# AiRyunn/BoT

Hardware: AMD Instinct MI355X
Metric: edges/sec full-batch GAT fwd+bwd on ogbn-arxiv; achieved HBM GB/s vs peak (higher is better)
Workload: dtype f32

## Files before the change

bot_amd/_C.py:

```python
from __future__ import annotations

import ctypes
import os
from ctypes import c_char_p, c_double, c_float, c_int32, c_int64, c_uint64, c_void_p

import torch

_HERE = os.path.dirname(os.path.abspath(__file__))
LIB_PATH = os.environ.get("BOT_AMD_LIB") or os.path.join(_HERE, "lib", "libbot_gnn.so")
ABI_VERSION = 19

if not os.path.exists(LIB_PATH):
    raise ImportError(
        f"{LIB_PATH} is missing: build the gfx950 kernels first "
        "(`make -C bot_amd/csrc` or `python -c 'import __graft_entry__ as g; g.build()'`). "
        "bot_amd has no CPU / PyTorch fallback."
    )
_lib = ctypes.CDLL(LIB_PATH)

_P = c_void_p
_SIGS = {
    "bot_abi_version": (ctypes.c_int, []),
    "bot_last_error": (c_char_p, []),
    "bot_last_kernel": (c_char_p, []),
# ... 88 lines not shown
                                                c_uint64, _P, _P, _P, c_double, _P, c_int64, _P, _P]),
    "bot_halves_tn_combine_f32": (ctypes.c_int, [_P, _P, c_int32, c_int32, c_int32, c_int32, _P, _P, _P, c_int64, _P]),
    "bot_halves_scale_from_slots2_f32": (ctypes.c_int, [_P, c_float, _P, c_float, _P, _P]),
    "bot_halves_tail_f16": (ctypes.c_int, [c_int64, c_int32, _P, _P, _P, _P, _P, c_int64, c_int32, _P]),
    "bot_spmm_dot_halves_fits": (ctypes.c_int, [_P, c_int64, c_int64, _P, c_int64, c_int64, c_int32, c_int32, _P, c_int64, c_int64, c_int32]),
    "bot_spmm_dot_halves_f16": (ctypes.c_int, [_P, _P, c_int64, c_int64, _P, c_int64, _P, _P, c_int64, _P, c_int64, c_int64, _P, _P, _P, c_int64, c_int64,
                                               c_int32, c_int32, _P, _P, c_int64, c_int64, c_int32, _P, _P, _P]),
    "bot_gemm_halves3_nt_bn_rows": (c_int32, [c_int64]),
    "bot_gemm_halves3_nt3_f32": (ctypes.c_int, [c_int64, c_int64, c_int64, _P, _P, c_int64, _P, _P, c_int64, c_int64, _P, c_int64, c_int64, c_int32, _P, c_int64,
                                                _P, c_int32, _P]),
    "bot_gemm_halves3_nt_bn_deferred_max_k": (c_int32, []),
    "bot_gemm_halves3_nt_bn_reduce_f32": (ctypes.c_int, [c_int64, c_int64, c_int64, _P, _P, c_int64, _P, _P, c_int64, c_int64, _P, c_int64, c_int64, c_int32, _P, c_int64,
                                                         _P, _P]),
    "bot_gemm_halves3_nt_bn_apply_f32": (ctypes.c_int, [c_int64, c_int64, c_int64, _P, _P, c_int64, _P, _P, c_int64, c_int64, _P, c_int64, c_int64, c_int32, _P,
                                                        _P, _P, c_double, _P, c_int64, _P, _P, c_int64, c_int32, c_int32, c_int32, _P, _P]),
    "bot_bn_act_bwd_reduce_partials_f32": (ctypes.c_int, [_P, c_int32, c_int32, _P, _P, _P]),
    "bot_bn_bwd_bound_partials_f32": (ctypes.c_int, [c_int32, _P, c_int32, _P, _P, c_double, _P, _P, _P, _P]),
    "bot_bn_bwd_partials_finish_f32": (ctypes.c_int, [_P, _P, c_int32, c_int32, _P, _P, c_int32, c_double, _P, _P, _P, _P]),
    "bot_gemm_halves3_nt2_f32": (ctypes.c_int, [c_int64, c_int64, c_int64, _P, _P, c_int64, _P, _P, c_int64, c_int64, _P, c_int64, c_int64, c_int32, _P, c_int64,
                                                c_int32, _P]),
    "bot_halves_split_frag_f16": (ctypes.c_int, [_P, c_int64, c_int64, c_int32, _P, _P, c_int32, _P]),
    "bot_gemm_halves3_tn2_f32": (ctypes.c_int, [c_int64, c_int64, c_int64, c_int64, c_int64, _P, _P, _P, c_int64, _P, c_int64, c_int64, _P, c_int64, c_int64, _P,
                                                c_int64, _P, c_int32, _P]),
    "bot_stream_create": (ctypes.c_int, [c_int32, _P]),
    "bot_gemm_halves3_nt_grouped2_f32": (ctypes.c_int, [c_int64, c_int64, _P, _P, _P, c_int64, c_int64, _P, c_int64, c_int64, _P, c_int64, c_int32, _P,
                                                        c_int32, _P, _P, c_int32, _P, _P, _P, _P, c_int32, c_int32, _P]),
    "bot_bn_stats_halves_partials_f32": (ctypes.c_int, [_P, _P, c_int32, _P, c_int64, c_int32, c_float, c_float, _P, _P, _P, _P, _P, _P, _P, c_float, _P, _P, _P]),
    "bot_absmax_slots": (c_int32, []),
    "bot_absmax_slots_f32": (ctypes.c_int, [_P, c_int64, c_int64, c_int32, _P, _P]),
    "bot_halves_scale_from_slots_f32": (ctypes.c_int, [_P, _P, _P]),
# ... 841 lines not shown
        n = b.shape[0]
    if out is None:
        out = torch.empty((m, n), dtype=torch.float32, device=a.device)
    st = None
    if bn is not None:
        if not bn.fits(m, n, k):
            raise BotKernelError("gemm_halves3_nt: this product cannot carry the BatchNorm-backward by-product (BnBwdStats.fits)")
        st = bn.struct()
    _check(_timed("gemm_halves", (m, n, 3 * k, 1), lambda: _lib.bot_gemm_halves3_nt3_f32(
        m, n, k, scale_a.data_ptr(), _ptr(scale_a2), int(k_split), scale_b.data_ptr(), a.data_ptr(), _ld(a), 2 * piece_a if a2_off is None else a2_off,
        b.data_ptr(), _ld(b), piece_b, int(bool(b_frag)), out.data_ptr(), _ld(out), ctypes.addressof(st) if st is not None else None, int(mode), _stream())),
        "gemm_halves3_nt")
    return out


def dh_deferred_max_k() -> int:
    return int(_lib.bot_gemm_halves3_nt_bn_deferred_max_k())


def gemm_halves3_nt_bn_reduce(a, b, scale_a, scale_b, piece_b, k, bn, a2_off, scale_a2=None, k_split=0, b_frag=False, n=None, out=None):
    _dev(a, b, scale_a, scale_b, scale_a2, out)
    m = a.shape[0]
    n = b.shape[0] if n is None else n
    st = bn.struct()
    _check(_timed("gemm_halves", (m, n, 3 * k, 1), lambda: _lib.bot_gemm_halves3_nt_bn_reduce_f32(
        m, n, k, scale_a.data_ptr(), _ptr(scale_a2), int(k_split), scale_b.data_ptr(), a.data_ptr(), _ld(a), a2_off, b.data_ptr(), _ld(b), piece_b,
        int(bool(b_frag)), _ptr(out), _ld(out) if out is not None else 0, ctypes.addressof(st), _stream())), "gemm_halves3_nt_bn_reduce")


def gemm_halves3_nt_bn_apply(a, b, scale_a, scale_b, piece_b, k, bn, a2_off, sum_g, sum_gx, total_count, scale_a2=None, k_split=0, b_frag=False, n=None,
# ... 813 lines not shown
```

bot_amd/csrc/dense.hip:

```cpp
#include <hip/hip_fp16.h>

#include "common.h"

#include <stdlib.h>

namespace bot {

constexpr int kTX = 64;
constexpr int kTY = 4;
constexpr int kRowBlocks = 256;

template <int VEC>
__device__ __forceinline__ void drop_factors(uint64_t seed, int64_t r, int c, int64_t nquad, float p, float scale, float (&f)[VEC]) {
    uint32_t w[4];
    Philox::gen(seed, (uint64_t)(r * nquad + (c >> 2)), w);
#pragma unroll
    for (int t = 0; t < VEC; ++t) f[t] = ((w[(c & 3) + t] >> 8) * (1.0f / 16777216.0f)) >= p ? scale : 0.f;
}

template <int VEC>
__device__ __forceinline__ void load_cols(float (&v)[VEC], const float* p, bool wide, int nv) {
    if constexpr (VEC == 4) {
        if (wide && nv == 4) {
            vload<4>(v, p);
        } else {
            const float2 a = *reinterpret_cast<const float2*>(p);
            v[0] = a.x, v[1] = a.y, v[2] = 0.f, v[3] = 0.f;
            if (nv == 4) {
                const float2 b = *reinterpret_cast<const float2*>(p + 2);
                v[2] = b.x, v[3] = b.y;
            }
        }
    } else {
        vload<VEC>(v, p);
    }
}
template <int VEC>
__device__ __forceinline__ void store_cols(float* p, const float (&v)[VEC], bool wide, int nv) {
    if constexpr (VEC == 4) {
        if (wide && nv == 4) {
            vstore<4>(p, v);
        } else {
            *reinterpret_cast<float2*>(p) = make_float2(v[0], v[1]);
            if (nv == 4) *reinterpret_cast<float2*>(p + 2) = make_float2(v[2], v[3]);
        }
    } else {
        vstore<VEC>(p, v);
    }
}
template <int VEC>
__device__ __forceinline__ void load_param(float (&v)[VEC], const float* a, int c, int F, float dflt) {
#pragma unroll
    for (int t = 0; t < VEC; ++t) v[t] = (a && c + t < F) ? a[c + t] : dflt;
}

__device__ __forceinline__ uint64_t eff_seed(uint64_t seed, const uint64_t* off) {
    return off ? seed + off[0] * 0x9E3779B97F4A7C15ull : seed;
}

struct BnArgs {
    const float* x;
    int64_t ldx;
    int64_t n;
    int32_t F;
    const float* mean;
    const float* invstd;
    const float* w;
    const float* b;
    int32_t relu;
    float p;
    uint64_t seed;
    const uint64_t* seed_offset;
    __half* hout;
    int32_t hpieces;
// ... 267 lines not shown
    const int64_t step = (int64_t)gridDim.y * kTY;
    for (int64_t r0 = (int64_t)blockIdx.y * kTY + ty; r0 < a.n; r0 += step * UR) {
        float v[UR][VEC];
#pragma unroll
        for (int u = 0; u < UR; ++u) {
            const int64_t r = r0 + u * step;
            if (r < a.n) load_cols<VEC>(v[u], a.x + r * a.ldx + c, a.wx, nv);
        }
#pragma unroll
        for (int u = 0; u < UR; ++u) {
            const int64_t r = r0 + u * step;
            if (r >= a.n) break;
            float f[VEC];
            if (a.p > 0.f) drop_factors<VEC>(seed, r, c, nquad, a.p, scale, f);
#pragma unroll
            for (int t = 0; t < VEC; ++t) {
                float o = fmaf(v[u][t] - mu[t], sc[t], sh[t]);
                if (a.relu) o = fmaxf(o, 0.f);
                if (a.p > 0.f) o *= f[t];
                v[u][t] = o;
            }
            if (a.y) store_cols<VEC>(a.y + r * a.ldy + c, v[u], a.wy, nv);
            if constexpr (VEC == 4) {
                if (a.hout) {
                    __half h1[4], h2[4];
#pragma unroll
                    for (int t = 0; t < 4; ++t) {
                        const float z = t < nv ? v[u][t] * hs : 0.f;
                        h1[t] = __float2half_rn(z);
                        h2[t] = __float2half_rn((z - __half2float(h1[t])) * kHalvesShift);
                    }
                    __half* o = a.hout + r * a.ldh + c;
                    const uint2 hi = *reinterpret_cast<const uint2*>(h1), lo = *reinterpret_cast<const uint2*>(h2);
                    *reinterpret_cast<uint2*>(o) = hi;
                    if (a.hpieces == 3) *reinterpret_cast<uint2*>(o + a.piece) = hi, *reinterpret_cast<uint2*>(o + 2 * (int64_t)a.piece) = lo;
                    else *reinterpret_cast<uint2*>(o + a.piece) = lo;
                }
            }
        }
    }
}

constexpr int kRowSeg = 8;
__global__ __launch_bounds__(256) void bn_act_fwd_rowseg_kernel(BnArgs a) {
    const int c = threadIdx.x * 4;
    if (c >= a.piece) return;
// ... 12 lines not shown
    const uint64_t seed = eff_seed(a.seed, a.seed_offset);
    const int64_t r0 = (int64_t)blockIdx.x * kRowSeg;
    float v[kRowSeg][4];
#pragma unroll
    for (int u = 0; u < kRowSeg; ++u)
        if (live && r0 + u < a.n) load_cols<4>(v[u], a.x + (r0 + u) * a.ldx + c, a.wx, nv);
#pragma unroll
    for (int u = 0; u < kRowSeg; ++u) {
        const int64_t r = r0 + u;
        if (r >= a.n) break;
        __half h1[4], h2[4];
        float f[4];
        if (live && a.p > 0.f) drop_factors<4>(seed, r, c, nquad, a.p, scale, f);
#pragma unroll
        for (int t = 0; t < 4; ++t) {
            float o = 0.f;
            if (t < nv) {
                o = fmaf(v[u][t] - mu[t], sc[t], sh[t]);
                if (a.relu) o = fmaxf(o, 0.f);
                if (a.p > 0.f) o *= f[t];
            }
            const float z = o * hs;
            h1[t] = __float2half_rn(z);
            h2[t] = __float2half_rn((z - __half2float(h1[t])) * kHalvesShift);
            v[u][t] = o;
        }
        if (a.y && live) store_cols<4>(a.y + r * a.ldy + c, v[u], a.wy, nv);
        __half* o = a.hout + r * a.ldh + c;
        const uint2 hi = *reinterpret_cast<const uint2*>(h1), lo = *reinterpret_cast<const uint2*>(h2);
        *reinterpret_cast<uint2*>(o) = hi;
        if (a.hpieces == 3) *reinterpret_cast<uint2*>(o + a.piece) = hi, *reinterpret_cast<uint2*>(o + 2 * (int64_t)a.piece) = lo;
        else *reinterpret_cast<uint2*>(o + a.piece) = lo;
    }
}

template <int VEC>
__global__ __launch_bounds__(kTX* kTY) void bn_act_bwd_reduce_kernel(BnArgs a) {
    __shared__ float lds[2][kTY][kTX * VEC];
    const int tx = threadIdx.x % kTX, ty = threadIdx.x / kTX;
// ... 605 lines not shown
```

bot_amd/csrc/halves3.hip:

```cpp
#include <hip/hip_fp16.h>

#include <stdlib.h>
#include <string.h>

#include <algorithm>
#include <type_traits>
#include <utility>

#include "common.h"

namespace bot {
namespace {

constexpr int BK = 32;

typedef _Float16 half8 __attribute__((ext_vector_type(8)));
typedef float f32x4 __attribute__((ext_vector_type(4)));

struct H3Args {
    const _Float16* A;
    const _Float16* B;
    const float* scale_a;
    const float* scale_b;
    float* C;
// ... 749 lines not shown
                    if (e < b_nv) pm[e] = b_gm[e], pm[F + e] = b_xm[e];
            }
        }
    }
}

__global__ __launch_bounds__(512) void gemm_halves3_nt64_kernel(H3Args p) { gemm_halves3_nt64_body<false, false>(p, nullptr); }
__global__ __launch_bounds__(512) void gemm_halves3_nt64_frag_kernel(H3Args p) { gemm_halves3_nt64_body<false, true>(p, nullptr); }
__global__ __launch_bounds__(512) void gemm_halves3_nt64_grouped_kernel(H3Args p, H3Groups groups) { gemm_halves3_nt64_body<true, false>(p, &groups); }
__global__ __launch_bounds__(512) void gemm_halves3_nt64_bnb_kernel(H3Args p) { gemm_halves3_nt64_body<false, false, kBnbStore>(p, nullptr); }
__global__ __launch_bounds__(512) void gemm_halves3_nt64_frag_bnb_kernel(H3Args p) { gemm_halves3_nt64_body<false, true, kBnbStore>(p, nullptr); }
__global__ __launch_bounds__(512) void gemm_halves3_nt64_bnreduce_kernel(H3Args p) { gemm_halves3_nt64_body<false, false, kBnbReduce>(p, nullptr); }
__global__ __launch_bounds__(512) void gemm_halves3_nt64_frag_bnreduce_kernel(H3Args p) { gemm_halves3_nt64_body<false, true, kBnbReduce>(p, nullptr); }
__global__ __launch_bounds__(512) void gemm_halves3_nt64_bnapply_kernel(H3Args p) { gemm_halves3_nt64_body<false, false, kBnbApply>(p, nullptr); }
__global__ __launch_bounds__(512) void gemm_halves3_nt64_frag_bnapply_kernel(H3Args p) { gemm_halves3_nt64_body<false, true, kBnbApply>(p, nullptr); }

static bool nt64_wanted() {
    static const bool wanted = [] {
        const char* e = getenv("BOT_NT_KERNEL");
        return !(e && !strcmp(e, "128x64"));
    }();
    return wanted;
}

constexpr int TBK = 32;
constexpr int TT = 192;
constexpr int kTnSubA = TBK * 256, kTnSubB = TBK * 128;
constexpr int kTnPiece = kTnSubA + kTnSubB;
constexpr int kTnStage = 4 * kTnPiece;
constexpr int kTnStages = 3;
// ... 438 lines not shown
    BOT_REQUIRE(dx || hout, BOT_E_NULL, "gemm_halves3_nt_bn_apply: neither dx nor hout");
    BOT_REQUIRE((sum_g == nullptr) == (sum_gx == nullptr), BOT_E_NULL, "gemm_halves3_nt_bn_apply: sum_g and sum_gx go together");
    BOT_REQUIRE(sum_g == nullptr || total_count >= 1.0, BOT_E_RANGE, "gemm_halves3_nt_bn_apply: total_count=%f", total_count);
    BOT_REQUIRE(dx == nullptr || (lddx >= n && lddx % 2 == 0 && aligned(dx, 8)), BOT_E_RANGE, "gemm_halves3_nt_bn_apply: dx rows must be 8-byte aligned, pitch >= n");
    BOT_REQUIRE(hout == nullptr || hscale, BOT_E_NULL, "gemm_halves3_nt_bn_apply: hout without hscale");
    BOT_REQUIRE(hout == nullptr || (hD >= 2 && hD % 2 == 0 && hDP >= hD && hDP % 2 == 0 && n % hD == 0 && h2_off % 2 == 0 && ldh % 2 == 0 &&
                                    h2_off >= (n / hD) * hDP && ldh >= h2_off + (n / hD) * hDP && aligned(hout, 4)),
                BOT_E_RANGE, "gemm_halves3_nt_bn_apply: F=%lld hD=%d hDP=%d h2_off=%d ldh=%lld", (long long)n, hD, hDP, h2_off, (long long)ldh);
    H3Args ap{};
    ap.ap_sum_g = sum_g, ap.ap_sum_gx = sum_gx, ap.ap_inv_count = sum_g ? (float)(1.0 / total_count) : 0.f, ap.ap_dx = dx, ap.ap_lddx = lddx;
    ap.ap_hscale = hscale, ap.ap_hout = reinterpret_cast<_Float16*>(hout), ap.ap_ldh = ldh, ap.ap_h2off = h2_off, ap.ap_hD = hout ? hD : 2, ap.ap_hDP = hout ? hDP : 2;
    ap.absmax = absmax_slots;
    return nt3_run(m, n, k, scale_a, scale_a2, k_split, scale_b, A, lda, a2_off, B, ldb, b2_off, b_layout, nullptr, 0, bn, 0, stream, kBnbApply, &ap);
}

extern "C" int bot_gemm_halves3_nt_grouped_f32(int64_t m, int64_t b_rows, const float* scale_a, const float* scale_b, const uint16_t* A, int64_t lda,
                                               int64_t a2_off, const uint16_t* B, int64_t ldb, int64_t b2_off, float* C, int64_t ldc, int32_t n_groups,
                                               const int64_t* groups, int32_t k_seg, const float* col_scale, const float* col_shift, int32_t relu,
                                               uint32_t* absmax_slots, int32_t mode, bot_stream_t stream) {
    return bot_gemm_halves3_nt_grouped2_f32(m, b_rows, scale_a, scale_b, A, lda, a2_off, B, ldb, b2_off, C, ldc, n_groups, groups, k_seg, col_scale, col_shift,
                                            relu, absmax_slots, nullptr, nullptr, nullptr, 0, mode, stream);
}

extern "C" int bot_gemm_halves3_nt_grouped2_f32(int64_t m, int64_t b_rows, const float* scale_a, const float* scale_b, const uint16_t* A, int64_t lda,
                                                int64_t a2_off, const uint16_t* B, int64_t ldb, int64_t b2_off, float* C, int64_t ldc, int32_t n_groups,
                                                const int64_t* groups, int32_t k_seg, const float* col_scale, const float* col_shift, int32_t relu,
                                                uint32_t* absmax_slots, float* stats_part, float* stats_minmax, float* stats_pivot, int32_t stats_F,
                                                int32_t mode, bot_stream_t stream) {
    using namespace bot;
    BOT_REQUIRE((stats_part == nullptr) == (stats_minmax == nullptr) && (stats_part == nullptr) == (stats_pivot == nullptr) && (stats_part == nullptr || stats_F >= 1), -1,
// ... 152 lines not shown
```

bot_amd/gemm.py:

```python
from __future__ import annotations

import os
import weakref

import torch

from . import _C

MODE = os.environ.get("BOT_GEMM", "halves")
NT_KERNEL = os.environ.get("BOT_GEMM_NT", "halves3")
TN_KERNEL = os.environ.get("BOT_GEMM_TN", "halves3")
LEFT_NODUP = NT_KERNEL == "halves3" and TN_KERNEL == "halves3" and os.environ.get("BOT_HALVES_DUP", "0") != "1"
NODUP_MIN_PIECE = int(os.environ.get("BOT_NODUP_MIN_PIECE", "256"))
TN_MIN_OUT = 512 * 1024
NT_MIN_COLS = 192
LINEAR_BLOCKS = os.environ.get("BOT_LINEAR_BLOCKS", "1") != "0"
FORCE = False
MIN_ROWS = 8192
PIECE_ALIGN = 64
SHIFT = 2048.0
CHUNK_ROWS = 8192


def enabled(x) -> bool:
# ... 29 lines not shown

    def __init__(self, st, a, scale_a, a2_off, k, b, scale_a2=None, k_split=0):
        self.st, self.a, self.scale_a, self.a2_off, self.k, self.b, self.scale_a2, self.k_split = st, a, scale_a, a2_off, k, b, scale_a2, k_split

    def _kw(self):
        return dict(a2_off=self.a2_off, scale_a2=self.scale_a2, k_split=self.k_split, b_frag=self.b.order == 3, n=self.b.n)

    def product(self):
        return _C.gemm_halves3_nt(self.a, self.b.buf, self.scale_a, self.b.scale, self.k, self.b.piece, self.k, **self._kw())

    def apply(self, sum_g, sum_gx, total, **out):
        return _C.gemm_halves3_nt_bn_apply(self.a, self.b.buf, self.scale_a, self.b.scale, self.b.piece, self.k, self.st, self.a2_off, sum_g, sum_gx, total,
                                           scale_a2=self.scale_a2, k_split=self.k_split, b_frag=self.b.order == 3, n=self.b.n, **out)


class BnLink:
    __slots__ = ("x", "mean", "invstd", "w", "b", "p", "seed", "relu", "sync", "stats", "key", "ref", "deferred")

    def __init__(self, x, mean, invstd, w, b, p, seed, relu=True, sync=False):
        self.x, self.mean, self.invstd, self.w, self.b, self.p, self.seed, self.relu = x, mean, invstd, w, b, p, seed, bool(relu)
        self.sync = bool(sync)
        self.stats = self.key = self.ref = self.deferred = None

    def stats_for(self, m, n, k):
        if not BN_BYPRODUCT or self.x is None:
            return None
        st = _C.BnBwdStats(self.x, self.mean, self.invstd, self.w, self.b, self.relu, self.p, self.seed)
        return st if st.fits(m, n, k) else None

    def deliver(self, st, dh, deferred=None):
# ... 105 lines not shown


_SCALES = {}


def stash_scale(y, scale):
    _SCALES.clear()
    _SCALES[(y.data_ptr(), y._version, tuple(y.shape))] = (weakref.ref(y), scale)


def split_with_stash(x, order: int) -> Halves:
    ref, scale = _SCALES.pop((x.data_ptr(), x._version, tuple(x.shape)), (None, None))
    return split(x, order, scale=scale if (scale is not None and ref() is not None) else None)


def take(x, order: int):
    ref, h = _STASH.pop((x.data_ptr(), x._version, tuple(x.shape)), (None, None))
    if h is not None and ref() is not None and h.left == (order != 1):
        STATS["taken"] += 1
        return h
    if is_handle(x):
        raise RuntimeError("bot_amd.gemm.take: this hidden state exists only as fp16 halves and they are no longer stashed "
                           "(it was produced for exactly one halves-GEMM consumer); set BOT_SKIP_Y=0 to store fp32 hidden states")
    STATS["split"] += 1
    return split(x, order)


def epilogue_piece(F: int, x) -> int | None:
    if MODE != "halves" or not (FORCE or (x.is_cuda and x.shape[0] >= MIN_ROWS)) or F % 2 or x.stride(0) % 2:
        return None
    return (F + PIECE_ALIGN - 1) // PIECE_ALIGN * PIECE_ALIGN


def _alpha(a: Halves, b: Halves, n=None):
    if n is None:
        return a.scale[1:] * b.scale[1:]
    return torch.mul(a.scale[1:].expand(n), b.scale[1:].expand(n))


def mm_nt(a: Halves, b: Halves, out=None, link: BnLink | None = None):
    assert a.left and b.order in (1, 3) and a.F == b.F and a.piece == b.piece
    if NT_KERNEL == "halves3" and (b.order == 3 or b.n >= NT_MIN_COLS or a.order == 2):
        st = link.stats_for(a.n, b.n, a.piece) if (link is not None and out is None) else None
        res = _C.gemm_halves3_nt(a.buf, b.buf, a.scale, b.scale, a.piece, b.piece, a.piece, out=out, a2_off=a.h2_off, b_frag=b.order == 3, n=b.n, bn=st)
        if st is not None:
            link.deliver(st, res)
        return res
    assert a.order == 0 and b.order == 1
    return _C.gemm_halves(a.buf, b.buf, _alpha(a, b, b.n), trans_b=True, out=out)


TN_NARROW = os.environ.get("BOT_GEMM_TN_NARROW", "1") != "0"
_TN_TILES = {}


def _tn_tiles(K: int, P: int):
# ... 127 lines not shown
```

bot_amd/nn/fused.py:

```python
from __future__ import annotations

import os
from types import SimpleNamespace

import torch
import torch.nn as nn
import torch.nn.functional as F

from .. import _C, gemm, halo, side
from ..graph import take_rows
from ..ops import bn_epilogue_forward, bn_epilogue_sums, new_dropout_seed, stats_partials_for


ABSMAX_BYPRODUCT = os.environ.get("BOT_ABSMAX_BYPRODUCT", "1") != "0"
SKIP_Y = os.environ.get("BOT_SKIP_Y", "1") != "0"
HANDLES = 0
SKINNY = os.environ.get("BOT_SKINNY", "1") != "0"
FORCE = False
CALLS = 0
AGG_CALLS = 0
L0_CALLS = 0


def can_fuse(conv, norm, activation, graph, training, stack_residual) -> bool:
# ... 185 lines not shown
            and g.number_of_dst_nodes() == h.shape[0]
            and HD % 2 == 0 and H >= 2 and c % 32 == 0 and P % 64 == 0 and gemm.left_order(P) == 2
            and gemm.NT_KERNEL == "halves3" and gemm.TN_KERNEL == "halves3" and (ctx.halves[2] * P >= gemm.TN_MIN_OUT or gemm.FORCE or FORCE) and not epi.sync)


class _GATHidden(torch.autograd.Function):
    @staticmethod
    def forward(ctx, h, Wcat, bn_w, bn_b, graph, bn, H, D, has_res, has_er, slope, attn_p, drop_p, bn_training, kp, sym, y_needed=True):
        N, HD = graph.number_of_dst_nodes(), H * D
        csc = graph.csc
        ctx.cfg, ctx.graph = (H, D, has_res, has_er, slope), graph
        ctx.sym = sym
        ctx.kp = kp
        xh = None
        if gemm.enabled(h):
            xh = gemm.take(h, 0)
            ws = gemm.split_right(Wcat.t().contiguous() if kp else Wcat)
            ctx.wscale = ws.scale
            ctx.xscale = xh.scale
            out = gemm.mm_nt(xh, ws)
        else:
            out = torch.mm(h, Wcat) if kp else torch.mm(h, Wcat.t())
        ctx.halves = None if xh is None else (xh.n, xh.F, xh.piece, xh.order)
        ctx.bn_link = None if xh is None else xh.bn_link
        ctx.h_handle = xh is not None and gemm.is_handle(h)
        hk = h if xh is None else xh.buf
        B = block_width(HD)
        c = 2 * B if has_res else B
        ext = None
        ctx.overlap = halo.enabled(graph) and not sym
        if ctx.overlap:
# ... 733 lines not shown
```

bot_amd/ops.py:

```python
from __future__ import annotations

import os
from collections import namedtuple

import torch

from . import _C
from .graph import take_rows

__all__ = ["copy_u_sum", "u_mul_e_sum", "copy_e_sum", "copy_u", "u_add_v", "edge_softmax", "gat_attention", "copy_u_max", "gatv2_logits"]


def _as3(x):
    if x.dim() == 1:
        return x.view(-1, 1, 1)
    if x.dim() == 2:
        return x.unsqueeze(1)
    if x.dim() == 3:
        return x
    return _flat2(x).unsqueeze(1)


def _flat2(t):
    w = 1
# ... 383 lines not shown

BnEpilogue = namedtuple("BnEpilogue", "drop_p seed bn_training sync group total out_link")


def bn_epilogue_forward(x, bn, weight, bias, relu, p, bn_training, halves, link, y_needed=True, partials=None):
    from . import gemm
    seed = new_dropout_seed(p)
    piece = gemm.epilogue_piece(x.shape[1], x) if halves and bn_training else None
    hscale = out_link = None
    if piece is not None:
        mean, invstd, total, sync, group, hscale = bn_batch_stats(x, bn, bn_training, halves_p=p, partials=partials)
    else:
        mean, invstd, total, sync, group = bn_batch_stats(x, bn, bn_training)
    if hscale is not None:
        order = gemm.left_order(piece)
        y, buf = _C.bn_act_fwd(x, mean, invstd, weight, bias, relu, p, seed, halves=(hscale, piece, 2 if order == 2 else 3), want_y=y_needed)
        if y is None:
            y = gemm.make_handle(x, x.shape[0], x.shape[1])
        hv = gemm.Halves(buf, hscale, x.shape[0], x.shape[1], piece, order)
        hv.bn_link = out_link = gemm.BnLink(x, mean, invstd, weight, bias, p, seed, relu=relu, sync=sync) if (link and gemm.BN_BYPRODUCT) else None
        gemm.stash(y, hv)
    else:
        y = _C.bn_act_fwd(x, mean, invstd, weight, bias, relu, p, seed)
    return y, mean, invstd, BnEpilogue(p, seed, bn_training, sync, group, total, out_link)


def bn_epilogue_sums(epi, dy, x, mean, invstd, weight, bias, relu, all_reduce, slots=None):
    import torch.distributed as dist
    train, total = epi.bn_training, epi.total
    st = epi.out_link.claim(dy) if epi.out_link is not None else None
    if st is not None and slots is not None and not all_reduce:
        sg, sgx = st.finish(train, total, slots)
        return ((sg, sgx) if train else (None, None)), (sg, sgx)
    if st is not None:
# ... 126 lines not shown
```

include/bot_gnn.h:

```cpp
#ifndef BOT_GNN_H
#define BOT_GNN_H

#include <stdint.h>

#ifdef __cplusplus
extern "C" {
#endif

#define BOT_ABI_VERSION 19

#define BOT_E_NULL (-1)
#define BOT_E_RANGE (-2)
#define BOT_E_ALIGN (-3)
#define BOT_E_PLAN (-4)

typedef void* bot_stream_t;

int bot_abi_version(void);
const char* bot_last_error(void);
int bot_stream_create(int32_t high_priority, bot_stream_t* out);
const char* bot_last_kernel(void);
int bot_debug_abort_trace(const char* path_host);

int bot_row_plan_size_host(const int32_t* indptr_host, int64_t n_rows, int32_t chunk,
// ... 294 lines not shown
    float* pmax;
} bot_bn_bwd_stats_t;
int32_t bot_gemm_halves3_nt_bn_rows(int64_t k);
int bot_gemm_halves3_nt3_f32(int64_t m, int64_t n, int64_t k, const float* scale_a, const float* scale_a2, int64_t k_split, const float* scale_b,
                             const uint16_t* A, int64_t lda, int64_t a2_off, const uint16_t* B, int64_t ldb, int64_t b2_off, int32_t b_layout, float* C,
                             int64_t ldc, const bot_bn_bwd_stats_t* bn, int32_t mode, bot_stream_t stream);
int32_t bot_gemm_halves3_nt_bn_deferred_max_k(void);
int bot_gemm_halves3_nt_bn_reduce_f32(int64_t m, int64_t n, int64_t k, const float* scale_a, const float* scale_a2, int64_t k_split, const float* scale_b,
                                      const uint16_t* A, int64_t lda, int64_t a2_off, const uint16_t* B, int64_t ldb, int64_t b2_off, int32_t b_layout,
                                      float* C, int64_t ldc, const bot_bn_bwd_stats_t* bn, bot_stream_t stream);
int bot_gemm_halves3_nt_bn_apply_f32(int64_t m, int64_t n, int64_t k, const float* scale_a, const float* scale_a2, int64_t k_split, const float* scale_b,
                                     const uint16_t* A, int64_t lda, int64_t a2_off, const uint16_t* B, int64_t ldb, int64_t b2_off, int32_t b_layout,
                                     const bot_bn_bwd_stats_t* bn, const float* sum_g, const float* sum_gx, double total_count, float* dx, int64_t lddx,
                                     const float* hscale, uint16_t* hout, int64_t ldh, int32_t h2_off, int32_t hD, int32_t hDP, uint32_t* absmax_slots,
                                     bot_stream_t stream);
int bot_bn_act_bwd_reduce_partials_f32(const float* part, int32_t nblk, int32_t F, float* sum_g, float* sum_gx, bot_stream_t stream);
int bot_bn_bwd_bound_partials_f32(int32_t F, const float* pmax, int32_t nblk, const float* sum_g, const float* sum_gx, double total_count,
                                  const float* weight, const float* invstd, uint32_t* absmax_slots, bot_stream_t stream);
int bot_bn_bwd_partials_finish_f32(const float* part, const float* pmax, int32_t nblk, int32_t F, float* sum_g, float* sum_gx, int32_t batch_stats,
                                   double total_count, const float* weight, const float* invstd, uint32_t* absmax_slots, bot_stream_t stream);
int bot_halves_split_frag_f16(const float* x, int64_t ldx, int64_t n, int32_t F, const float* scale, uint16_t* out, int32_t piece, bot_stream_t stream);
int bot_gemm_halves3_tn2_f32(int64_t n_rows, int64_t k, int64_t p, int64_t kp, int64_t pp, const float* scale_x, const float* scale_d, const float* scale_d2,
                             int64_t p_split, const uint16_t* X, int64_t ldx, int64_t x2_off, const uint16_t* D, int64_t ldd, int64_t d2_off, float* out,
                             int64_t ldo, float* workspace, int32_t mode, bot_stream_t stream);

int bot_gemm_halves3_nt_grouped_f32(int64_t m, int64_t b_rows, const float* scale_a, const float* scale_b, const uint16_t* A, int64_t lda,
                                    int64_t a2_off, const uint16_t* B, int64_t ldb, int64_t b2_off, float* C, int64_t ldc, int32_t n_groups,
                                    const int64_t* groups, int32_t k_seg, const float* col_scale, const float* col_shift, int32_t relu,
                                    uint32_t* absmax_slots, int32_t mode, bot_stream_t stream);
int bot_gemm_halves3_nt_grouped2_f32(int64_t m, int64_t b_rows, const float* scale_a, const float* scale_b, const uint16_t* A, int64_t lda,
// ... 47 lines not shown
```

Baseline: 245.6 million.

## Fuse BN+activation+dropout+halves split into the following NT GEMM prologue

Adds a fused kernel that applies batch-norm, ReLU and dropout to the fp32 input, splits the result into fp16 halves in LDS, and runs the halves3 NT product in the same launch. The half buffer is still written for backward use. The BN forward output becomes a deferred operand that is only materialized when a consumer cannot use the fused projection. This removes one separate elementwise launch and the global round trip of the halves buffer before the GEMM. The cost is a more complex GEMM prologue and lower occupancy, since waves per EU are capped at 2.

```diff
diff --git a/bot_amd/_C.py b/bot_amd/_C.py
--- a/bot_amd/_C.py
+++ b/bot_amd/_C.py
@@ -126,6 +126,8 @@
                                                          _P, _P]),
     "bot_gemm_halves3_nt_bn_apply_f32": (ctypes.c_int, [c_int64, c_int64, c_int64, _P, _P, c_int64, _P, _P, c_int64, c_int64, _P, c_int64, c_int64, c_int32, _P,
                                                         _P, _P, c_double, _P, c_int64, _P, _P, c_int64, c_int32, c_int32, c_int32, _P, _P]),
+    "bot_gemm_halves3_nt_bn_fwd_f32": (ctypes.c_int, [_P, c_int64, c_int64, c_int32, _P, _P, _P, _P, c_int32, c_float, c_uint64, _P, _P, _P, c_int64, c_int32,
+                                                      c_int32, c_int64, _P, _P, c_int64, c_int64, c_int32, _P, c_int64, _P]),
     "bot_bn_act_bwd_reduce_partials_f32": (ctypes.c_int, [_P, c_int32, c_int32, _P, _P, _P]),
     "bot_bn_bwd_bound_partials_f32": (ctypes.c_int, [c_int32, _P, c_int32, _P, _P, c_double, _P, _P, _P, _P]),
     "bot_bn_bwd_partials_finish_f32": (ctypes.c_int, [_P, _P, c_int32, c_int32, _P, _P, c_int32, c_double, _P, _P, _P, _P]),
@@ -997,6 +999,31 @@
     return out
 
 
+BN_PROJECT_MAX_N, BN_PROJECT_MAX_PIECE = 128, 1024
+
+
+def bn_project_fits(x, n, piece) -> bool:
+    F = x.shape[1]
+    return (x.is_cuda and x.dim() == 2 and x.dtype == torch.float32 and x.stride(1) == 1 and F % 2 == 0 and x.stride(0) % 2 == 0 and x.data_ptr() % 8 == 0
+            and 1 <= n <= BN_PROJECT_MAX_N and piece == (F + 63) // 64 * 64 and piece <= BN_PROJECT_MAX_PIECE)
+
+
+def gemm_halves3_nt_bn_fwd(x, mean, invstd, weight, bias, relu, p, seed, hscale, piece, pieces, b, scale_b, piece_b, n, b_frag=False, out=None):
+    _dev(x, mean, invstd, hscale, b, scale_b)
+    x = _mat(x, "x")
+    m, F = x.shape
+    if not bn_project_fits(x, n, piece):
+        raise BotKernelError(f"gemm_halves3_nt_bn_fwd: x {tuple(x.shape)} / n={n} / piece={piece} is outside what the fused launch serves (bn_project_fits)")
+    buf = torch.empty((m, pieces * piece), dtype=torch.float16, device=x.device)
+    if out is None:
+        out = torch.empty((m, n), dtype=torch.float32, device=x.device)
+    _check(_timed("bn_project", (F, n), lambda: _lib.bot_gemm_halves3_nt_bn_fwd_f32(
+        x.data_ptr(), x.stride(0), m, F, mean.data_ptr(), invstd.data_ptr(), _ptr(weight), _ptr(bias), int(relu), float(p), int(seed), _seed_off(p),
+        hscale.data_ptr(), buf.data_ptr(), buf.stride(0), piece, pieces, n, scale_b.data_ptr(), b.data_ptr(), _ld(b), piece_b, int(bool(b_frag)),
+        out.data_ptr(), _ld(out), _stream())), "gemm_halves3_nt_bn_fwd")
+    return out, buf
+
+
 def dh_deferred_max_k() -> int:
     return int(_lib.bot_gemm_halves3_nt_bn_deferred_max_k())
 
diff --git a/bot_amd/csrc/bn_act.h b/bot_amd/csrc/bn_act.h
--- /dev/null
+++ b/bot_amd/csrc/bn_act.h
@@ -0,0 +1,57 @@
+#pragma once
+#include <hip/hip_fp16.h>
+
+#include "common.h"
+
+namespace bot {
+
+template <int VEC>
+__device__ __forceinline__ void drop_factors(uint64_t seed, int64_t r, int c, int64_t nquad, float p, float scale, float (&f)[VEC]) {
+    uint32_t w[4];
+    Philox::gen(seed, (uint64_t)(r * nquad + (c >> 2)), w);
+#pragma unroll
+    for (int t = 0; t < VEC; ++t) f[t] = ((w[(c & 3) + t] >> 8) * (1.0f / 16777216.0f)) >= p ? scale : 0.f;
+}
+
+template <int VEC>
+__device__ __forceinline__ void load_cols(float (&v)[VEC], const float* p, bool wide, int nv) {
+    if constexpr (VEC == 4) {
+        if (wide && nv == 4) {
+            vload<4>(v, p);
+        } else {
+            const float2 a = *reinterpret_cast<const float2*>(p);
+            v[0] = a.x, v[1] = a.y, v[2] = 0.f, v[3] = 0.f;
+            if (nv == 4) {
+                const float2 b = *reinterpret_cast<const float2*>(p + 2);
+                v[2] = b.x, v[3] = b.y;
+            }
+        }
+    } else {
+        vload<VEC>(v, p);
+    }
+}
+template <int VEC>
+__device__ __forceinline__ void load_param(float (&v)[VEC], const float* a, int c, int F, float dflt) {
+#pragma unroll
+    for (int t = 0; t < VEC; ++t) v[t] = (a && c + t < F) ? a[c + t] : dflt;
+}
+
+__device__ __forceinline__ uint64_t eff_seed(uint64_t seed, const uint64_t* off) {
+    return off ? seed + off[0] * 0x9E3779B97F4A7C15ull : seed;
+}
+
+__device__ __forceinline__ float bn_act_fwd_value(float x, float mu, float sc, float sh, bool relu, bool drop, float f) {
+#pragma clang fp contract(off)
+    float o = fmaf(x - mu, sc, sh);
+    if (relu) o = fmaxf(o, 0.f);
+    if (drop) o *= f;
+    return o;
+}
+
+__device__ __forceinline__ void halves_left_split(float v, float hs, __half& h1, __half& h2) {
+#pragma clang fp contract(off)
+    h1 = __float2half_rn(v * hs);
+    h2 = __float2half_rn(fmaf(v, hs, -__half2float(h1)) * kHalvesShift);
+}
+
+}
diff --git a/bot_amd/csrc/dense.hip b/bot_amd/csrc/dense.hip
--- a/bot_amd/csrc/dense.hip
+++ b/bot_amd/csrc/dense.hip
@@ -1,5 +1,6 @@
 #include <hip/hip_fp16.h>
 
+#include "bn_act.h"
 #include "common.h"
 
 #include <stdlib.h>
@@ -10,31 +11,6 @@
 constexpr int kTY = 4;
 constexpr int kRowBlocks = 256;
 
-template <int VEC>
-__device__ __forceinline__ void drop_factors(uint64_t seed, int64_t r, int c, int64_t nquad, float p, float scale, float (&f)[VEC]) {
-    uint32_t w[4];
-    Philox::gen(seed, (uint64_t)(r * nquad + (c >> 2)), w);
-#pragma unroll
-    for (int t = 0; t < VEC; ++t) f[t] = ((w[(c & 3) + t] >> 8) * (1.0f / 16777216.0f)) >= p ? scale : 0.f;
-}
-
-template <int VEC>
-__device__ __forceinline__ void load_cols(float (&v)[VEC], const float* p, bool wide, int nv) {
-    if constexpr (VEC == 4) {
-        if (wide && nv == 4) {
-            vload<4>(v, p);
-        } else {
-            const float2 a = *reinterpret_cast<const float2*>(p);
-            v[0] = a.x, v[1] = a.y, v[2] = 0.f, v[3] = 0.f;
-            if (nv == 4) {
-                const float2 b = *reinterpret_cast<const float2*>(p + 2);
-                v[2] = b.x, v[3] = b.y;
-            }
-        }
-    } else {
-        vload<VEC>(v, p);
-    }
-}
 template <int VEC>
 __device__ __forceinline__ void store_cols(float* p, const float (&v)[VEC], bool wide, int nv) {
     if constexpr (VEC == 4) {
@@ -48,16 +24,6 @@
         vstore<VEC>(p, v);
     }
 }
-template <int VEC>
-__device__ __forceinline__ void load_param(float (&v)[VEC], const float* a, int c, int F, float dflt) {
-#pragma unroll
-    for (int t = 0; t < VEC; ++t) v[t] = (a && c + t < F) ? a[c + t] : dflt;
-}
-
-__device__ __forceinline__ uint64_t eff_seed(uint64_t seed, const uint64_t* off) {
-    return off ? seed + off[0] * 0x9E3779B97F4A7C15ull : seed;
-}
-
 struct BnArgs {
     const float* x;
     int64_t ldx;
@@ -355,22 +321,13 @@
             float f[VEC];
             if (a.p > 0.f) drop_factors<VEC>(seed, r, c, nquad, a.p, scale, f);
 #pragma unroll
-            for (int t = 0; t < VEC; ++t) {
-                float o = fmaf(v[u][t] - mu[t], sc[t], sh[t]);
-                if (a.relu) o = fmaxf(o, 0.f);
-                if (a.p > 0.f) o *= f[t];
-                v[u][t] = o;
-            }
+            for (int t = 0; t < VEC; ++t) v[u][t] = bn_act_fwd_value(v[u][t], mu[t], sc[t], sh[t], a.relu, a.p > 0.f, f[t]);
             if (a.y) store_cols<VEC>(a.y + r * a.ldy + c, v[u], a.wy, nv);
             if constexpr (VEC == 4) {
                 if (a.hout) {
                     __half h1[4], h2[4];
 #pragma unroll
-                    for (int t = 0; t < 4; ++t) {
-                        const float z = t < nv ? v[u][t] * hs : 0.f;
-                        h1[t] = __float2half_rn(z);
-                        h2[t] = __float2half_rn((z - __half2float(h1[t])) * kHalvesShift);
-                    }
+                    for (int t = 0; t < 4; ++t) halves_left_split(t < nv ? v[u][t] : 0.f, hs, h1[t], h2[t]);
                     __half* o = a.hout + r * a.ldh + c;
                     const uint2 hi = *reinterpret_cast<const uint2*>(h1), lo = *reinterpret_cast<const uint2*>(h2);
                     *reinterpret_cast<uint2*>(o) = hi;
@@ -413,15 +370,8 @@
         if (live && a.p > 0.f) drop_factors<4>(seed, r, c, nquad, a.p, scale, f);
 #pragma unroll
         for (int t = 0; t < 4; ++t) {
-            float o = 0.f;
-            if (t < nv) {
-                o = fmaf(v[u][t] - mu[t], sc[t], sh[t]);
-                if (a.relu) o = fmaxf(o, 0.f);
-                if (a.p > 0.f) o *= f[t];
-            }
-            const float z = o * hs;
-            h1[t] = __float2half_rn(z);
-            h2[t] = __float2half_rn((z - __half2float(h1[t])) * kHalvesShift);
+            const float o = t < nv ? bn_act_fwd_value(v[u][t], mu[t], sc[t], sh[t], a.relu, a.p > 0.f, f[t]) : 0.f;
+            halves_left_split(o, hs, h1[t], h2[t]);
             v[u][t] = o;
         }
         if (a.y && live) store_cols<4>(a.y + r * a.ldy + c, v[u], a.wy, nv);
diff --git a/bot_amd/csrc/halves3.hip b/bot_amd/csrc/halves3.hip
--- a/bot_amd/csrc/halves3.hip
+++ b/bot_amd/csrc/halves3.hip
@@ -7,6 +7,7 @@
 #include <type_traits>
 #include <utility>
 
+#include "bn_act.h"
 #include "common.h"
 
 namespace bot {
@@ -787,6 +788,207 @@
 __global__ __launch_bounds__(512) void gemm_halves3_nt64_frag_bnreduce_kernel(H3Args p) { gemm_halves3_nt64_body<false, true, kBnbReduce>(p, nullptr); }
 __global__ __launch_bounds__(512) void gemm_halves3_nt64_bnapply_kernel(H3Args p) { gemm_halves3_nt64_body<false, false, kBnbApply>(p, nullptr); }
 __global__ __launch_bounds__(512) void gemm_halves3_nt64_frag_bnapply_kernel(H3Args p) { gemm_halves3_nt64_body<false, true, kBnbApply>(p, nullptr); }
+
+struct BnFwdNtArgs {
+    const float* x;
+    int64_t ldx;
+    int M, F;
+    const float* mean;
+    const float* invstd;
+    const float* w;
+    const float* b;
+    int relu;
+    float p;
+    uint64_t seed;
+    const uint64_t* seed_offset;
+    const float* scale_a;
+    _Float16* hout;
+    int64_t ldh;
+    int piece, pieces;
+    const _Float16* B;
+    int64_t ldb;
+    int b2_off;
+    const float* scale_b;
+    float* C;
+    int64_t ldc;
+    int N;
+    bool wx;
+};
+
+template <bool BFRAG, bool WX>
+__global__ __launch_bounds__(256) __attribute__((amdgpu_waves_per_eu(2, 2))) void gemm_halves3_nt_bn_fwd_kernel(BnFwdNtArgs p) {
+    constexpr int BM = 128, MT = BM / 16, NT = 2;
+    constexpr int kRow = 4 * BK;
+    constexpr int kABytes = BM * kRow;
+    constexpr int kStageBytes = 2 * kABytes, kStages = 2;
+    constexpr int kPass = BM / 16;
+    constexpr int kMaxPiece = 1024;
+    __shared__ __attribute__((aligned(1024))) unsigned char lds[kStages * kStageBytes];
+    __shared__ __attribute__((aligned(16))) float par[3][kMaxPiece];
+    const int tid = threadIdx.x, lane = tid & 63, w = __builtin_amdgcn_readfirstlane(tid >> 6);
+    const int m0 = blockIdx.x * BM;
+    const int Tk = p.piece / BK, T2 = Tk >> 1;
+    const float alpha = p.scale_a[1] * p.scale_b[1];
+    const float hs = p.scale_a[0];
+    const int ntiles = (p.N + 15) >> 4;
+    const int nact = max(0, min(NT, ntiles - w * NT));
+
+    const int q = tid & 15, lrow = tid >> 4;
+    const bool drop = p.p > 0.f;
+    const float keep = drop ? 1.f / (1.f - p.p) : 1.f;
+    const int64_t nquad = (p.F + 3) / 4;
+    const uint64_t seed = eff_seed(p.seed, p.seed_offset);
+    for (int c = tid; c < p.piece; c += 256) {
+        float mu[1], sc[1], sh[1], wv[1];
+        load_param<1>(mu, p.mean, c, p.F, 0.f);
+        load_param<1>(sc, p.invstd, c, p.F, 0.f);
+        load_param<1>(wv, p.w, c, p.F, 1.f);
+        load_param<1>(sh, p.b, c, p.F, 0.f);
+        par[0][c] = mu[0], par[1][c] = sc[0] * wv[0], par[2][c] = sh[0];
+    }
+    auto load_x = [&](f32x4 (&xq)[kPass], int it) {
+        const int c = it * 64 + q * 4;
+        const int nv = max(0, min(4, p.F - c));
+        const float* xp = p.x + (int64_t)(m0 + lrow) * p.ldx + c;
+#pragma unroll
+        for (int u = 0; u < kPass; ++u) {
+            const bool in = m0 + u * 16 + lrow < p.M;
+            xq[u] = f32x4{0.f, 0.f, 0.f, 0.f};
+            const float* xr = xp + (int64_t)(u * 16) * p.ldx;
+            if (WX && in && nv == 4) {
+                xq[u] = *reinterpret_cast<const f32x4*>(xr);
+            } else if (in && nv > 0) {
+                const float2 lo = *reinterpret_cast<const float2*>(xr);
+                xq[u][0] = lo.x, xq[u][1] = lo.y;
+                if (nv == 4) {
+                    const float2 hi = *reinterpret_cast<const float2*>(xr + 2);
+                    xq[u][2] = hi.x, xq[u][3] = hi.y;
+                }
+            }
+        }
+    };
+    auto make_a = [&](const f32x4 (&xq)[kPass], int it, int stage) {
+        const int c = it * 64 + q * 4;
+        const int nv = max(0, min(4, p.F - c));
+        const f32x4 mu = *reinterpret_cast<const f32x4*>(&par[0][c]), sc = *reinterpret_cast<const f32x4*>(&par[1][c]);
+        const f32x4 sh = *reinterpret_cast<const f32x4*>(&par[2][c]);
+        unsigned char* st = lds + stage * kStageBytes;
+#pragma unroll
+        for (int u = 0; u < kPass; ++u) {
+            const int r = u * 16 + lrow, row = m0 + r;
+            __half h1[4], h2[4];
+            float f[4] = {1.f, 1.f, 1.f, 1.f};
+            if (nv > 0 && drop && row < p.M) drop_factors<4>(seed, (int64_t)row, c, nquad, p.p, keep, f);
+#pragma unroll
+            for (int t = 0; t < 4; ++t) {
+                const float o = (t < nv && row < p.M) ? bn_act_fwd_value(xq[u][t], mu[t], sc[t], sh[t], p.relu, drop, f[t]) : 0.f;
+                halves_left_split(o, hs, h1[t], h2[t]);
+            }
+            const uint2 hi = *reinterpret_cast<const uint2*>(h1), lo = *reinterpret_cast<const uint2*>(h2);
+            const int off = r * kRow + (((q >> 1) ^ ((r >> 1) & 7)) * 16) + (q & 1) * 8;
+            *reinterpret_cast<uint2*>(st + off) = hi;
+            *reinterpret_cast<uint2*>(st + kABytes + off) = lo;
+            if (row < p.M) {
+                _Float16* o = p.hout + (int64_t)row * p.ldh + c;
+                *reinterpret_cast<uint2*>(o) = hi;
+                if (p.pieces == 3) *reinterpret_cast<uint2*>(o + p.piece) = hi, *reinterpret_cast<uint2*>(o + 2 * (int64_t)p.piece) = lo;
+                else *reinterpret_cast<uint2*>(o + p.piece) = lo;
+            }
+            __builtin_amdgcn_sched_barrier(0);
+        }
+    };
+
+    uint32_t offB[NT];
+    int tileoff[NT];
+#pragma unroll
+    for (int nt = 0; nt < NT; ++nt) {
+        if constexpr (BFRAG) {
+            offB[nt] = lane * 16;
+            tileoff[nt] = min(w * NT + nt, ntiles - 1) * Tk * 1024;
+        } else {
+            offB[nt] = ((uint32_t)min(w * (NT * 16) + nt * 16 + (lane & 15), p.N - 1) * (uint32_t)p.ldb) * 2 + (lane >> 4) * 16;
+            tileoff[nt] = 0;
+        }
+    }
+    const int b2 = BFRAG ? ntiles * Tk * 1024 : p.b2_off * 2;
+    auto load_b = [&](half8 (&x1)[NT], half8 (&x2)[NT], int it, int sub) {
+#pragma unroll
+        for (int nt = 0; nt < NT; ++nt) {
+            const int so = BFRAG ? tileoff[nt] + (2 * it + sub) * 1024 : it * kRow + sub * 64;
+            if (nt >= nact) continue;
+            x1[nt] = load16(p.B, offB[BFRAG ? 0 : nt], so);
+            x2[nt] = load16(p.B, offB[BFRAG ? 0 : nt], so + b2);
+        }
+    };
+    const int frow = lane & 15, fkey = (frow >> 1) & 7;
+    const int a_off_s[2] = {frow * kRow + (((lane >> 4) ^ fkey) * 16), frow * kRow + (((4 + (lane >> 4)) ^ fkey) * 16)};
+
+    f32x4 acc[MT][NT];
+#pragma unroll
+    for (int mt = 0; mt < MT; ++mt)
+#pragma unroll
+        for (int nt = 0; nt < NT; ++nt) acc[mt][nt] = f32x4{0.f, 0.f, 0.f, 0.f};
+    const _Float16 sh11 = (_Float16)(1.0f / kHalvesShift);
+
+    half8 b1[2][NT] = {}, b2h[2][NT] = {};
+    f32x4 xa[kPass];
+    load_x(xa, 0);
+    load_b(b1[0], b2h[0], 0, 0);
+    load_b(b1[1], b2h[1], 0, 1);
+    __syncthreads();
+    auto iteration = [&](f32x4 (&xq)[kPass], int it) {
+        const int stage = it & 1;
+        make_a(xq, it, stage);
+        if (it + 1 < T2) load_x(xq, it + 1);
+        asm volatile("s_waitcnt lgkmcnt(0)" ::: "memory");
+        __builtin_amdgcn_s_barrier();
+        asm volatile("" ::: "memory");
+        const unsigned char* st = lds + stage * kStageBytes;
+#pragma unroll
+        for (int sub = 0; sub < 2; ++sub) {
+            half8 bs[NT];
+#pragma unroll
+            for (int nt = 0; nt < NT; ++nt) bs[nt] = b1[sub][nt] * sh11;
+#pragma unroll
+            for (int mt = 0; mt < MT; ++mt) {
+                const half8 a1 = *reinterpret_cast<const half8*>(st + a_off_s[sub] + mt * 2048);
+                const half8 a2 = *reinterpret_cast<const half8*>(st + a_off_s[sub] + mt * 2048 + kABytes);
+#pragma unroll
+                for (int nt = 0; nt < NT; ++nt)
+                    if (nt < nact) {
+                        acc[mt][nt] = __builtin_amdgcn_mfma_f32_16x16x32_f16(b1[sub][nt], a1, acc[mt][nt], 0, 0, 0);
+                        acc[mt][nt] = __builtin_amdgcn_mfma_f32_16x16x32_f16(b2h[sub][nt], a1, acc[mt][nt], 0, 0, 0);
+                        acc[mt][nt] = __builtin_amdgcn_mfma_f32_16x16x32_f16(bs[nt], a2, acc[mt][nt], 0, 0, 0);
+                    }
+            }
+        }
+        if (it + 1 < T2) {
+            load_b(b1[0], b2h[0], it + 1, 0);
+            load_b(b1[1], b2h[1], it + 1, 1);
+        }
+    };
+    for (int it = 0; it < T2; ++it) iteration(xa, it);
+
+    const bool vec_ok = (p.ldc % 4 == 0) && ((reinterpret_cast<uintptr_t>(p.C) & 15) == 0);
+#pragma unroll
+    for (int mt = 0; mt < MT; ++mt) {
+        const int row = m0 + mt * 16 + (lane & 15);
+#pragma unroll
+        for (int nt = 0; nt < NT; ++nt) {
+            const int col = w * (NT * 16) + nt * 16 + (lane >> 4) * 4;
+            if (nt >= nact || row >= p.M || col >= p.N) continue;
+            const f32x4 v = acc[mt][nt] * alpha;
+            float* c = p.C + (int64_t)row * p.ldc + col;
+            if (vec_ok && col + 3 < p.N) {
+                *reinterpret_cast<float4*>(c) = make_float4(v[0], v[1], v[2], v[3]);
+            } else {
+#pragma unroll
+                for (int e = 0; e < 4; ++e)
+                    if (col + e < p.N) c[e] = v[e];
+            }
+        }
+    }
+}
 
 static bool nt64_wanted() {
     static const bool wanted = [] {
@@ -1255,6 +1457,36 @@
     return nt3_run(m, n, k, scale_a, scale_a2, k_split, scale_b, A, lda, a2_off, B, ldb, b2_off, b_layout, nullptr, 0, bn, 0, stream, kBnbApply, &ap);
 }
 
+extern "C" int bot_gemm_halves3_nt_bn_fwd_f32(const float* x, int64_t ldx, int64_t m, int32_t F, const float* mean, const float* invstd, const float* weight,
+                                              const float* bias, int32_t relu, float p, uint64_t seed, const uint64_t* seed_offset, const float* scale_a,
+                                              uint16_t* hout, int64_t ldh, int32_t piece, int32_t pieces, int64_t n, const float* scale_b, const uint16_t* B,
+                                              int64_t ldb, int64_t b2_off, int32_t b_layout, float* C, int64_t ldc, bot_stream_t stream) {
+    using namespace bot;
+    BOT_REQUIRE(m >= 0 && m < (1ll << 31) - 256 && F >= 2 && F % 2 == 0 && ldx >= F && ldx % 2 == 0, BOT_E_RANGE,
+                "gemm_halves3_nt_bn_fwd: m=%lld F=%d ldx=%lld (an even F and 8-byte aligned x rows)", (long long)m, F, (long long)ldx);
+    BOT_REQUIRE(p >= 0.f && p < 1.f, BOT_E_RANGE, "gemm_halves3_nt_bn_fwd: dropout p=%f must be in [0,1)", (double)p);
+    BOT_REQUIRE(n >= 1 && n <= 128 && piece >= 64 && piece <= 1024 && piece % 64 == 0 && piece == (F + 63) / 64 * 64, BOT_E_RANGE,
+                "gemm_halves3_nt_bn_fwd: serves n <= 128 output columns and piece = F rounded up to x64 <= 1024 (n=%lld F=%d piece=%d)", (long long)n, F, piece);
+    if (m == 0) return 0;
+    BOT_REQUIRE(x && mean && invstd && scale_a && scale_b && hout && B && C, BOT_E_NULL, "gemm_halves3_nt_bn_fwd: NULL pointer");
+    BOT_REQUIRE(aligned(x, 8) && (pieces == 2 || pieces == 3) && ldh >= pieces * (int64_t)piece && ldh % 4 == 0 && aligned(hout, 8) && ldc >= n, BOT_E_ALIGN,
+                "gemm_halves3_nt_bn_fwd: x / hout rows must be 8-byte aligned, ldh >= pieces * piece (ldh=%lld pieces=%d), ldc >= n", (long long)ldh, pieces);
+    BOT_REQUIRE(aligned(B, 16) && (b_layout == 1 || (b_layout == 0 && ldb % 8 == 0 && b2_off % 8 == 0 && b2_off + piece <= ldb)), BOT_E_ALIGN,
+                "gemm_halves3_nt_bn_fwd: the right operand must be 16-byte aligned, row-major with b2_off + piece <= ldb or fragment-major (b_layout 1)");
+    BnFwdNtArgs a{};
+    a.x = x, a.ldx = ldx, a.M = (int)m, a.F = F, a.mean = mean, a.invstd = invstd, a.w = weight, a.b = bias, a.relu = relu, a.p = p, a.seed = seed;
+    a.seed_offset = seed_offset, a.scale_a = scale_a, a.hout = reinterpret_cast<_Float16*>(hout), a.ldh = ldh, a.piece = piece, a.pieces = pieces;
+    a.B = reinterpret_cast<const _Float16*>(B), a.ldb = ldb, a.b2_off = (int)b2_off, a.scale_b = scale_b, a.C = C, a.ldc = ldc, a.N = (int)n;
+    a.wx = aligned(x, 16) && ldx % 4 == 0;
+    const dim3 grid((unsigned)((m + 127) / 128));
+    set_kernel(b_layout ? "bot::gemm_halves3_nt_bn_fwd_kernel<frag>" : "bot::gemm_halves3_nt_bn_fwd_kernel<rows>");
+    if (b_layout && a.wx) hipLaunchKernelGGL((gemm_halves3_nt_bn_fwd_kernel<true, true>), grid, dim3(256), 0, (hipStream_t)stream, a);
+    else if (b_layout) hipLaunchKernelGGL((gemm_halves3_nt_bn_fwd_kernel<true, false>), grid, dim3(256), 0, (hipStream_t)stream, a);
+    else if (a.wx) hipLaunchKernelGGL((gemm_halves3_nt_bn_fwd_kernel<false, true>), grid, dim3(256), 0, (hipStream_t)stream, a);
+    else hipLaunchKernelGGL((gemm_halves3_nt_bn_fwd_kernel<false, false>), grid, dim3(256), 0, (hipStream_t)stream, a);
+    return hip_status("gemm_halves3_nt_bn_fwd");
+}
+
 extern "C" int bot_gemm_halves3_nt_grouped_f32(int64_t m, int64_t b_rows, const float* scale_a, const float* scale_b, const uint16_t* A, int64_t lda,
                                                int64_t a2_off, const uint16_t* B, int64_t ldb, int64_t b2_off, float* C, int64_t ldc, int32_t n_groups,
                                                const int64_t* groups, int32_t k_seg, const float* col_scale, const float* col_shift, int32_t relu,
diff --git a/bot_amd/gemm.py b/bot_amd/gemm.py
--- a/bot_amd/gemm.py
+++ b/bot_amd/gemm.py
@@ -67,6 +67,44 @@
                                            scale_a2=self.scale_a2, k_split=self.k_split, b_frag=self.b.order == 3, n=self.b.n, **out)
 
 
+BN_PROJECT = os.environ.get("BOT_BN_PROJECT", "1") != "0"
+BN_PROJECT_CALLS = 0
+
+
+class DeferredOperand(Halves):
+    __slots__ = ("x", "mean", "invstd", "w", "b", "relu", "p", "seed")
+
+    def __init__(self, x, mean, invstd, w, b, relu, p, seed, scale, piece, order):
+        super().__init__(None, scale, x.shape[0], x.shape[1], piece, order)
+        self.x, self.mean, self.invstd, self.w, self.b, self.relu, self.p, self.seed = x, mean, invstd, w, b, relu, p, seed
+
+    @property
+    def pieces(self):
+        return 2 if self.order == 2 else 3
+
+    def _done(self, buf):
+        self.buf = buf
+        self.x = self.mean = self.invstd = self.w = self.b = None
+        return self
+
+    def materialize(self):
+        if self.buf is None:
+            _, buf = _C.bn_act_fwd(self.x, self.mean, self.invstd, self.w, self.b, self.relu, self.p, self.seed, halves=(self.scale, self.piece, self.pieces),
+                                   want_y=False)
+            self._done(buf)
+        return self
+
+    def project(self, b: Halves, out=None):
+        if self.buf is not None or not (NT_KERNEL == "halves3" and _C.bn_project_fits(self.x, b.n, self.piece)):
+            return None
+        global BN_PROJECT_CALLS
+        BN_PROJECT_CALLS += 1
+        res, buf = _C.gemm_halves3_nt_bn_fwd(self.x, self.mean, self.invstd, self.w, self.b, self.relu, self.p, self.seed, self.scale, self.piece, self.pieces,
+                                             b.buf, b.scale, b.piece, b.n, b_frag=b.order == 3, out=out)
+        self._done(buf)
+        return res
+
+
 class BnLink:
     __slots__ = ("x", "mean", "invstd", "w", "b", "p", "seed", "relu", "sync", "stats", "key", "ref", "deferred")
 
@@ -202,10 +240,12 @@
     return split(x, order, scale=scale if (scale is not None and ref() is not None) else None)
 
 
-def take(x, order: int):
+def take(x, order: int, deferred_ok: bool = False):
     ref, h = _STASH.pop((x.data_ptr(), x._version, tuple(x.shape)), (None, None))
     if h is not None and ref() is not None and h.left == (order != 1):
         STATS["taken"] += 1
+        if isinstance(h, DeferredOperand) and not deferred_ok:
+            h.materialize()
         return h
     if is_handle(x):
         raise RuntimeError("bot_amd.gemm.take: this hidden state exists only as fp16 halves and they are no longer stashed "
@@ -228,6 +268,11 @@
 
 def mm_nt(a: Halves, b: Halves, out=None, link: BnLink | None = None):
     assert a.left and b.order in (1, 3) and a.F == b.F and a.piece == b.piece
+    if isinstance(a, DeferredOperand) and a.buf is None:
+        res = a.project(b, out) if (link is None and (b.order == 3 or b.n >= NT_MIN_COLS or a.order == 2)) else None
+        if res is not None:
+            return res
+        a.materialize()
     if NT_KERNEL == "halves3" and (b.order == 3 or b.n >= NT_MIN_COLS or a.order == 2):
         st = link.stats_for(a.n, b.n, a.piece) if (link is not None and out is None) else None
         res = _C.gemm_halves3_nt(a.buf, b.buf, a.scale, b.scale, a.piece, b.piece, a.piece, out=out, a2_off=a.h2_off, b_frag=b.order == 3, n=b.n, bn=st)
diff --git a/bot_amd/nn/fused.py b/bot_amd/nn/fused.py
--- a/bot_amd/nn/fused.py
+++ b/bot_amd/nn/fused.py
@@ -223,7 +223,7 @@
         ctx.kp = kp
         xh = None
         if gemm.enabled(h):
-            xh = gemm.take(h, 0)
+            xh = gemm.take(h, 0, deferred_ok=True)
             ws = gemm.split_right(Wcat.t().contiguous() if kp else Wcat)
             ctx.wscale = ws.scale
             ctx.xscale = xh.scale
diff --git a/bot_amd/ops.py b/bot_amd/ops.py
--- a/bot_amd/ops.py
+++ b/bot_amd/ops.py
@@ -421,10 +421,14 @@
         mean, invstd, total, sync, group = bn_batch_stats(x, bn, bn_training)
     if hscale is not None:
         order = gemm.left_order(piece)
-        y, buf = _C.bn_act_fwd(x, mean, invstd, weight, bias, relu, p, seed, halves=(hscale, piece, 2 if order == 2 else 3), want_y=y_needed)
-        if y is None:
+        if gemm.BN_PROJECT and not y_needed and x.is_cuda and gemm.NT_KERNEL == "halves3" and piece <= _C.BN_PROJECT_MAX_PIECE:
             y = gemm.make_handle(x, x.shape[0], x.shape[1])
-        hv = gemm.Halves(buf, hscale, x.shape[0], x.shape[1], piece, order)
+            hv = gemm.DeferredOperand(x, mean, invstd, weight, bias, relu, p, seed, hscale, piece, order)
+        else:
+            y, buf = _C.bn_act_fwd(x, mean, invstd, weight, bias, relu, p, seed, halves=(hscale, piece, 2 if order == 2 else 3), want_y=y_needed)
+            if y is None:
+                y = gemm.make_handle(x, x.shape[0], x.shape[1])
+            hv = gemm.Halves(buf, hscale, x.shape[0], x.shape[1], piece, order)
         hv.bn_link = out_link = gemm.BnLink(x, mean, invstd, weight, bias, p, seed, relu=relu, sync=sync) if (link and gemm.BN_BYPRODUCT) else None
         gemm.stash(y, hv)
     else:
diff --git a/include/bot_gnn.h b/include/bot_gnn.h
--- a/include/bot_gnn.h
+++ b/include/bot_gnn.h
@@ -332,6 +332,10 @@
                                      const bot_bn_bwd_stats_t* bn, const float* sum_g, const float* sum_gx, double total_count, float* dx, int64_t lddx,
                                      const float* hscale, uint16_t* hout, int64_t ldh, int32_t h2_off, int32_t hD, int32_t hDP, uint32_t* absmax_slots,
                                      bot_stream_t stream);
+int bot_gemm_halves3_nt_bn_fwd_f32(const float* x, int64_t ldx, int64_t m, int32_t F, const float* mean, const float* invstd, const float* weight,
+                                   const float* bias, int32_t relu, float p, uint64_t seed, const uint64_t* seed_offset, const float* scale_a,
+                                   uint16_t* hout, int64_t ldh, int32_t piece, int32_t pieces, int64_t n, const float* scale_b, const uint16_t* B,
+                                   int64_t ldb, int64_t b2_off, int32_t b_layout, float* C, int64_t ldc, bot_stream_t stream);
 int bot_bn_act_bwd_reduce_partials_f32(const float* part, int32_t nblk, int32_t F, float* sum_g, float* sum_gx, bot_stream_t stream);
 int bot_bn_bwd_bound_partials_f32(int32_t F, const float* pmax, int32_t nblk, const float* sum_g, const float* sum_gx, double total_count,
                                   const float* weight, const float* invstd, uint32_t* absmax_slots, bot_stream_t stream);
```

Measured after the change: 245.5 million. No clear change (-0.0%).
